# yandex/pire

Hardware: AMD Instinct MI355X
Metric: scanned GB/s (whole node) + ns/byte, 8-regex glued Scanner, 4KiB strings (higher is better)
Workload: dtype u8

## Files before the change

pire_amd/csrc/segmented.hip:

```cpp

#include <hip/hip_runtime.h>
#include <hipcub/hipcub.hpp>

#include <algorithm>
#include <cmath>
#include <chrono>
#include <cstdio>
#include <cstdlib>
#include <string>
#include <unordered_map>
#include <vector>

#include "device_common.h"

namespace pirehip {

namespace {

constexpr uint32_t kMaxModes = 6;
constexpr uint32_t kSlots = kMaxModes + 1;
constexpr uint64_t kResetMap = 1ull << 56;
constexpr uint32_t kNoSlot = 0xFF;
constexpr uint32_t kNoState = 0xFFFFFFFFu;

struct SegGeometry {
	uint64_t segBytes, warmBytes;
	uint64_t nStrings, nSeg;
	uint64_t segsPerString;
	const uint32_t* strFirst;
};

struct SegArrays {
	uint64_t* segBegin;
	uint64_t* segEnd;
	uint64_t* warmBegin;
	uint32_t* segStr;
	uint32_t* segJ;
	uint32_t* initSeg;
};

struct SlotArrays {
	uint32_t* guess[kSlots];
	uint32_t* end[kSlots];
	uint32_t count;
};

struct ChainArrays {
	uint64_t* prefix;
	uint32_t* trueStart;
	uint32_t* finalState;
	uint32_t* strDone;
	uint32_t* breakSeg;
	uint32_t* breakState;
	uint32_t* broken;
	uint64_t* blockAgg;
	uint64_t* blockPrefix;
	uint32_t* brokenHost;
};

__device__ __forceinline__ void StringOfSegment(const SegGeometry& g, uint64_t seg, uint64_t* str, uint64_t* j)
{
	if (!g.strFirst) {
		*str = seg / g.segsPerString;
		*j = seg - *str * g.segsPerString;
		return;
	}
	uint64_t lo = 0, hi = g.nStrings;
	while (hi - lo > 1) {
		const uint64_t mid = (lo + hi) / 2;
		if (g.strFirst[mid] <= seg)
			lo = mid;
		else
			hi = mid;
	}
	*str = lo;
	*j = seg - g.strFirst[lo];
}

__global__ void SegmentPrepKernel(ScanParams p, SegGeometry g, SegArrays a, uint32_t* patchGuess, uint32_t* patchEnd,
                                  uint32_t* strDone, uint32_t* breakSeg, uint32_t* broken)
{
	const uint64_t seg = uint64_t(blockIdx.x) * blockDim.x + threadIdx.x;
	if (seg >= g.nSeg)
		return;
	patchGuess[seg] = kNoState;
	patchEnd[seg] = kNoState;
	if (seg < g.nStrings) {
		strDone[seg] = 0;
		breakSeg[seg] = kNoState;
	}
	if (seg == 0)
		*broken = 0;
	uint64_t s, j;
	StringOfSegment(g, seg, &s, &j);
	uint64_t B, E;
	if (p.offsets) {
		B = p.offsets[s];
		E = p.offsets[s + 1];
	} else {
		B = s * p.stride;
		E = B + p.len;
	}
	const uint64_t b = B + j * g.segBytes;
	const uint64_t e = b + g.segBytes < E ? b + g.segBytes : E;
	const uint64_t w = j == 0 ? 0 : (b - B < g.warmBytes ? b - B : g.warmBytes);
	a.segBegin[seg] = b;
	a.segEnd[seg] = e;
	a.warmBegin[seg] = b - w;
	a.segStr[seg] = uint32_t(s);
	a.segJ[seg] = uint32_t(j);
	if (a.initSeg)
		a.initSeg[seg] = p.permOfOrig[p.initIdx[s]];
}

__global__ void SegmentFillKernel(uint32_t* dst, uint32_t value, uint64_t n)
{
	const uint64_t i = uint64_t(blockIdx.x) * blockDim.x + threadIdx.x;
	if (i < n)
		dst[i] = value;
}

__device__ __forceinline__ uint64_t MapOfSegment(const SegGeometry& g, const SegArrays& a, const SlotArrays& sl, uint64_t k)
{
	const bool last = k + 1 == g.nSeg || a.segJ[k + 1] == 0;
	uint64_t map = 0;
	if (!last) {
		uint32_t nextGuess[kSlots];
#pragma unroll
		for (uint32_t j = 0; j < kSlots; ++j)
			nextGuess[j] = (j < sl.count || j == kMaxModes) ? sl.guess[j][k + 1] : kNoState;
#pragma unroll
		for (uint32_t i = 0; i < kSlots; ++i) {
			uint32_t to = kNoSlot;
			if (i < sl.count || i == kMaxModes) {
				const uint32_t e = sl.end[i][k];
				const bool live = sl.guess[i][k] != kNoState;
#pragma unroll
				for (uint32_t j = kSlots; j-- > 0;)
					if (live && nextGuess[j] == e)
						to = j;
			}
			map |= uint64_t(to) << (8 * i);
		}
	}
	if (a.segJ[k] == 0) {
		const uint64_t to0 = map & 0xFF;
		map = to0 * 0x0001010101010101ull | kResetMap;
	}
	return map;
}

struct ComposeMaps {
	__host__ __device__ __forceinline__ uint64_t operator()(const uint64_t& first, const uint64_t& then) const
	{
		if (then & kResetMap)
			return then;
		uint64_t out = first & kResetMap;
#pragma unroll
		for (uint32_t i = 0; i < kSlots; ++i) {
			const uint32_t mid = uint32_t(first >> (8 * i)) & 0xFF;
			const uint32_t to = mid == kNoSlot ? kNoSlot : uint32_t(then >> (8 * mid)) & 0xFF;
			out |= uint64_t(to) << (8 * i);
		}
		return out;
	}
};

constexpr uint32_t kChainBlock = 1024;
constexpr uint64_t kIdentityMap = 0x0006050403020100ull;

__global__ __launch_bounds__(kChainBlock) void SegmentMapScanKernel(SegGeometry g, SegArrays a, SlotArrays sl, ChainArrays c)
{
	using Scan = hipcub::BlockScan<uint64_t, kChainBlock>;
	__shared__ typename Scan::TempStorage temp;
	const uint64_t k = uint64_t(blockIdx.x) * kChainBlock + threadIdx.x;
	uint64_t map = kIdentityMap;
	if (k < g.nSeg)
		map = MapOfSegment(g, a, sl, k);
	uint64_t incl;
	Scan(temp).InclusiveScan(map, incl, ComposeMaps());
	if (k < g.nSeg)
		c.prefix[k] = incl;
	if (threadIdx.x == kChainBlock - 1)
		c.blockAgg[blockIdx.x] = incl;
}

__global__ __launch_bounds__(kChainBlock) void SegmentBlockScanKernel(ChainArrays c, uint32_t nblocks)
{
	using Scan = hipcub::BlockScan<uint64_t, kChainBlock>;
	__shared__ typename Scan::TempStorage temp;
	__shared__ uint64_t next;
	uint64_t carry = kIdentityMap;
	for (uint32_t base = 0; base < nblocks; base += kChainBlock) {
		const uint32_t b = base + threadIdx.x;
		const uint64_t agg = b < nblocks ? c.blockAgg[b] : kIdentityMap;
		uint64_t in;
		Scan(temp).InclusiveScan(agg, in, ComposeMaps());
		const uint64_t out = ComposeMaps()(carry, in);
		if (b < nblocks)
			c.blockPrefix[b] = out;
		if (threadIdx.x == kChainBlock - 1)
			next = out;
		__syncthreads();
		carry = next;
		__syncthreads();
	}
}

__device__ __forceinline__ uint32_t ChainSlotAfter(const ChainArrays& c, uint64_t k)
{
	const uint64_t local = c.prefix[k];
// ... 147 lines not shown
						w = SlowStep(p, lds, L, w, byte);
						take(w);
					});
					hs = w < p.hot ? w : p.hot;
					cold = w;
				}
			}
			st = hs != p.hot ? hs : cold;
		}
		for (; q < qe; ++q) {
			st = SlowStep(p, lds, L, st, *q);
			take(st);
		}
		const bool last = k + 1 == g.nSeg || a.segJ[k + 1] == 0;
		if (last && (p.flags & PIRE_HIP_RUN_END)) {
			st = p.nextPerm[size_t(st) * p.letters + p.endCls];
			take(st);
		}
		const uint32_t str = a.segStr[k];
#pragma unroll
		for (int r = 0; r < 8; ++r)
			if (uint32_t(r) < p.regexps && c[r]) {
				if (str == firstStr)
					atomicAdd(&blockSum[r], c[r]);
				else
					atomicAdd(&results[size_t(str) * p.regexps + r], c[r]);
			}
	}
	__syncthreads();
	if (threadIdx.x < p.regexps && threadIdx.x < 8 && blockSum[threadIdx.x])
		atomicAdd(&results[size_t(firstStr) * p.regexps + threadIdx.x], blockSum[threadIdx.x]);
}

__global__ __launch_bounds__(256) void SegmentFinishSmallKernel(ScanParams p, const uint32_t* endIdx, const uint32_t* broken,
                                                               uint32_t* brokenHost)
{
	if (!ChainsIntact(broken, brokenHost))
		return;
	const uint64_t s = uint64_t(blockIdx.x) * blockDim.x + threadIdx.x;
	const bool active = s < p.n;
	const FinRec* recs = (p.flags & PIRE_HIP_RUN_END) ? p.finEnd : p.finSelf;
	u32x4 raw = {0, 0, 0, 0};
	if (active)
		raw = *reinterpret_cast<const u32x4*>(&recs[endIdx[s]]);
	const uint32_t orig = raw.x, endPerm = raw.y & 0x0FFFFFFFu, fl = raw.y >> 28;
	if (active) {
		if (p.outIdx)
			p.outIdx[s] = orig;
		if (p.outFinal)
			p.outFinal[s] = fl & kFinal;
	}
	if (!p.outCounts)
		return;
	const int lane = threadIdx.x & 63;
	const unsigned long long finals = __ballot(active && (fl & kFinal));
	const unsigned long long actives = __ballot(active);
	if (lane == 0 && actives) {
		atomicAdd(&p.outCounts[0], (unsigned long long)__popcll(finals));
		atomicAdd(&p.outCounts[1], (unsigned long long)__popcll(actives));
	}
	if (p.acceptMaskPerm) {
		const uint64_t m = active ? ((uint64_t(raw.w) << 32) | raw.z) : 0;
		if (__any(m != 0))
			for (uint32_t r = 0; r < p.regexps; ++r) {
				const unsigned long long b = __ballot((m >> r) & 1);
				if (lane == 0 && b)
					atomicAdd(&p.outCounts[2 + r], (unsigned long long)__popcll(b));
			}
	} else if (active) {
		for (uint64_t k = p.acceptOffPerm[endPerm]; k < p.acceptOffPerm[endPerm + 1]; ++k)
			atomicAdd(&p.outCounts[2 + p.acceptIds[k]], 1ull);
	}
}

uint64_t Knob(uint64_t v, uint64_t fallback)
{
	return v == 0 ? fallback : v == ~uint64_t(0) ? 0 : v;
}

struct HostWord {
	void* host = nullptr;
	uint32_t* dev = nullptr;
	size_t block = 0;
	int Acquire()
	{
		if (int rc = StagingAcquireHost(64, &host, &block))
			return rc;
		void* d = nullptr;
		const hipError_t e = hipHostGetDevicePointer(&d, host, 0);
		if (e != hipSuccess)
			return HipFail(e, "hipHostGetDevicePointer");
		dev = static_cast<uint32_t*>(d);
		return PIRE_HIP_OK;
	}
	~HostWord()
	{
		if (host)
			StagingReleaseHost(host, block);
	}
};

struct ScratchArena {
	StreamScratch block;
	uint8_t* base = nullptr;
	size_t size = 0, used = 0;
// ... 209 lines not shown
		prod.ranked = false;
		t->segProductA.resize(PN);
		t->segProductB.resize(PN);
		for (uint32_t i = 0; i < PN; ++i) {
			t->segProductA[i] = pairs[i].first;
			t->segProductB[i] = pairs[i].second;
		}
		t->segProduct.reset(new pire_hip_table);
		t->segProduct->host = std::move(prod);
	}
	if (t->segProduct && t->segProductA0 == a0 && t->segProductB0 == b0) {
		out->table = t->segProduct.get();
		out->compA = &t->segProductA;
		out->compB = &t->segProductB;
	}
	return PIRE_HIP_OK;
}

__global__ void SegmentSplitKernel(const uint32_t* guessP, const uint32_t* endP, const uint32_t* compA, const uint32_t* compB,
                                   uint32_t productStates, const uint32_t* productOrigOfPerm, const uint32_t* permOfOrig,
                                   uint32_t* guessA, uint32_t* endA, uint32_t* guessB, uint32_t* endB, uint64_t n)
{
	const uint64_t k = uint64_t(blockIdx.x) * blockDim.x + threadIdx.x;
	if (k >= n)
		return;
	const uint32_t g = guessP[k], e = endP[k];
	const uint32_t go = g < productStates ? productOrigOfPerm[g] : kNoState, eo = e < productStates ? productOrigOfPerm[e] : kNoState;
	guessA[k] = go != kNoState ? permOfOrig[compA[go]] : kNoState;
	guessB[k] = go != kNoState ? permOfOrig[compB[go]] : kNoState;
	endA[k] = eo != kNoState ? permOfOrig[compA[eo]] : kNoState;
	endB[k] = eo != kNoState ? permOfOrig[compB[eo]] : kNoState;
}

bool SegmentedEligible(uint64_t n, uint64_t totalBytes)
{
	const pire_hip_config cfg = GetConfig();
	if (cfg.no_segments || n == 0 || n >= (1ull << 20))
		return false;
	if (cfg.segment_bytes)
		return true;
	const double mean = double(totalBytes) / double(n);
	if (mean < 8192.0)
		return false;
	const double lanes = 256.0 * 1024.0;
	const double plain = std::ceil(double(n) / lanes) * mean / 25e6;
	const double segmented = double(totalBytes) / 2.0e12 + 80e-6;
	return plain > 1.5 * segmented;
}

int RunSegmented(pire_hip_table* t, const ScanParams& p, const uint64_t* hostOffsets, hipStream_t stream,
                 uint32_t* halfFinalResults, bool* halfFinalIncomplete)
{
	PIRE_TRY(CheckCounts(p));
	const pire_hip_config cfg = GetConfig();
	const bool wantStats = cfg.segment_stats != 0;
	auto t0 = std::chrono::steady_clock::now();
	std::string timeline;
	auto mark = [&](const char* what) {
		if (!wantStats)
			return;
		(void)hipStreamSynchronize(stream);
		const auto t1 = std::chrono::steady_clock::now();
		char buf[64];
		snprintf(buf, sizeof(buf), " %s %.0f us;", what, std::chrono::duration<double, std::micro>(t1 - t0).count());
		timeline += buf;
		t0 = t1;
	};
	const uint64_t n = p.n;
	const uint64_t total = hostOffsets ? hostOffsets[n] - hostOffsets[0] : n * p.len;
	int cus = 0;
	PIRE_TRY(DeviceCUs(&cus));
	const uint64_t wanted = uint64_t(cus) * 1024;
	uint64_t segBytes = std::min<uint64_t>(1u << 20, std::max<uint64_t>(1024, (total / wanted + 255) / 256 * 256));
	segBytes = Knob(cfg.segment_bytes, segBytes);
	const uint64_t warmBytes = Knob(cfg.segment_warmup, 256);
	const uint32_t maxModes = uint32_t(std::min<uint64_t>(kMaxModes, std::max<uint64_t>(1, Knob(cfg.segment_modes, 6))));
	uint64_t budget = Knob(cfg.segment_budget, 32);
	if (segBytes == 0) {
		SetError("PIRE_HIP_SEGMENT_BYTES must be positive");
		return PIRE_HIP_EINVAL;
	}

	SegGeometry g = {};
	g.segBytes = segBytes;
	g.warmBytes = warmBytes;
	g.nStrings = n;
	std::vector<uint32_t> strFirst(n + 1);
	{
		uint64_t acc = 0;
		for (uint64_t i = 0; i < n; ++i) {
			strFirst[i] = uint32_t(acc);
			const uint64_t len = hostOffsets ? hostOffsets[i + 1] - hostOffsets[i] : p.len;
			acc += std::max<uint64_t>(1, (len + segBytes - 1) / segBytes);
			if (acc >= (1ull << 31)) {
				SetError("too many segments");
				return PIRE_HIP_EINVAL;
			}
		}
		strFirst[n] = uint32_t(acc);
		g.nSeg = acc;
	}
	const uint64_t S = g.nSeg;
	ScratchArena scratch(stream);
	const uint64_t chainBlocks = (S + kChainBlock - 1) / kChainBlock;
	{
		const size_t perSeg = 3 * 8 + 3 * 4
		                      + (size_t(maxModes) + 1) * 8 + 4
		                      + 8
		                      + 4;
		const size_t perString = 5 * 4 + 2 * 8 + 3 * 4 + 4;
		PIRE_TRY(scratch.Reserve(S * perSeg + n * perString + chainBlocks * 16 + size_t(t->host.states) * 4 * kMaxModes + 64 * 256));
	}
	if (hostOffsets) {
		uint32_t* d = nullptr;
		PIRE_TRY(scratch.Alloc(&d, n + 1));
		PIRE_TRY(HipOk(hipMemcpyAsync(d, strFirst.data(), (n + 1) * 4, hipMemcpyHostToDevice, stream), "hipMemcpy(segment index)"));
		g.strFirst = d;
	} else {
		g.segsPerString = strFirst[1] - strFirst[0];
	}
	SegArrays a = {};
	PIRE_TRY(scratch.Alloc(&a.segBegin, S));
	PIRE_TRY(scratch.Alloc(&a.segEnd, S));
	PIRE_TRY(scratch.Alloc(&a.warmBegin, S));
	PIRE_TRY(scratch.Alloc(&a.segStr, S));
	PIRE_TRY(scratch.Alloc(&a.segJ, S));
	if (p.initIdx)
		PIRE_TRY(scratch.Alloc(&a.initSeg, S));
	const unsigned blocks = unsigned((S + 255) / 256);
	SlotArrays sl = {};
	PIRE_TRY(scratch.Alloc(&sl.guess[kMaxModes], S));
	PIRE_TRY(scratch.Alloc(&sl.end[kMaxModes], S));
	ChainArrays c = {};
	PIRE_TRY(scratch.Alloc(&c.prefix, S));
	PIRE_TRY(scratch.Alloc(&c.blockAgg, chainBlocks));
	PIRE_TRY(scratch.Alloc(&c.blockPrefix, chainBlocks));
	if (halfFinalResults)
		PIRE_TRY(scratch.Alloc(&c.trueStart, S));
	PIRE_TRY(scratch.Alloc(&c.finalState, n));
	PIRE_TRY(scratch.Alloc(&c.strDone, n));
	PIRE_TRY(scratch.Alloc(&c.breakSeg, n));
	PIRE_TRY(scratch.Alloc(&c.breakState, n));
	PIRE_TRY(scratch.Alloc(&c.broken, 1));
	auto segBeginOf = [&](uint64_t i, uint32_t k) {
		const uint64_t B = hostOffsets ? hostOffsets[i] : i * p.stride;
		return B + uint64_t(k - strFirst[i]) * segBytes;
	};
	auto stringEndOf = [&](uint64_t i) { return hostOffsets ? hostOffsets[i + 1] : i * p.stride + p.len; };

	ScanParams q = p;
	q.len = q.stride = 0;
	q.textEnd = hostOffsets ? hostOffsets[n] : (n - 1) * p.stride + p.len;
	q.outFinal = nullptr;
	q.outCounts = nullptr;

	uint64_t gridSegs = 0;
	if (!hostOffsets && !cfg.segment_no_grid) {
		if (n == 1)
			gridSegs = p.len / segBytes;
		else if (p.stride == p.len && p.len % segBytes == 0)
			gridSegs = S;
		ScanParams probe = q;
		probe.offsets = nullptr;
		probe.n = gridSegs;
		probe.len = probe.stride = segBytes;
		if (!TiledEligible(probe))
			gridSegs = 0;
	}

	uint32_t* dConst = nullptr;
	const uint64_t fusedSegs = (warmBytes % 256 == 0 && warmBytes <= segBytes && segBytes % 256 == 0 && !cfg.segment_no_pair)
	                               ? gridSegs & ~uint64_t(63) : 0;
	auto addMode = [&](bool first, uint32_t representative) -> int {
		const uint32_t m = sl.count;
		PIRE_TRY(scratch.Alloc(&sl.guess[m], S));
		PIRE_TRY(scratch.Alloc(&sl.end[m], S));
		if (fusedSegs) {
			ScanParams r = q;
			r.offsets = nullptr;
			r.ends = nullptr;
			r.n = fusedSegs;
			r.len = r.stride = segBytes;
			r.outIdx = sl.end[m];
			if (first) {
				r.initIdx = a.initSeg;
				r.flags = (p.flags & PIRE_HIP_RUN_BEGIN) | kPermIds;
			} else {
				r.initIdx = nullptr;
				r.startPerm = representative;
				r.flags = kPermIds;
			}
			PIRE_TRY(LaunchTiledSeg(r, warmBytes, a.segJ, sl.guess[m], stream));
			if (fusedSegs < S) {
				const uint64_t rest = S - fusedSegs;
				if (!first) {
					if (!dConst)
						PIRE_TRY(scratch.Alloc(&dConst, S));
					hipLaunchKernelGGL(SegmentFillKernel, dim3(unsigned((rest + 255) / 256)), dim3(256), 0, stream, dConst, representative, rest);
				}
				q.n = rest;
				q.offsets = a.warmBegin + fusedSegs;
				q.ends = a.segBegin + fusedSegs;
				q.initIdx = first ? (a.initSeg ? a.initSeg + fusedSegs : nullptr) : dConst;
				q.flags = (first ? (p.flags & PIRE_HIP_RUN_BEGIN) : 0u) | kPermIds;
				q.outIdx = sl.guess[m] + fusedSegs;
				PIRE_TRY(ScanBatch(q, t, stream));
				q.flags = kPermIds;
				q.offsets = a.segBegin + fusedSegs;
				q.ends = a.segEnd + fusedSegs;
				q.initIdx = sl.guess[m] + fusedSegs;
				q.outIdx = sl.end[m] + fusedSegs;
				PIRE_TRY(ScanBatch(q, t, stream));
			}
			sl.count = m + 1;
			return PIRE_HIP_OK;
		}
		q.n = S;
		q.offsets = a.warmBegin;
		q.ends = a.segBegin;
		if (first) {
			q.initIdx = a.initSeg;
			q.flags = (p.flags & PIRE_HIP_RUN_BEGIN) | kPermIds;
		} else {
			if (!dConst)
				PIRE_TRY(scratch.Alloc(&dConst, S));
			hipLaunchKernelGGL(SegmentFillKernel, dim3(blocks), dim3(256), 0, stream, dConst, representative, S);
			q.initIdx = dConst;
			q.flags = kPermIds;
		}
		q.outIdx = sl.guess[m];
		PIRE_TRY(ScanBatch(q, t, stream));
		q.flags = kPermIds;
		if (gridSegs) {
			ScanParams r = q;
			r.offsets = nullptr;
			r.ends = nullptr;
			r.n = gridSegs;
			r.len = r.stride = segBytes;
			r.initIdx = sl.guess[m];
			r.outIdx = sl.end[m];
			PIRE_TRY(LaunchTiled(r, stream));
		}
		if (gridSegs < S) {
			q.n = S - gridSegs;
			q.offsets = a.segBegin + gridSegs;
			q.ends = a.segEnd + gridSegs;
			q.initIdx = sl.guess[m] + gridSegs;
			q.outIdx = sl.end[m] + gridSegs;
			PIRE_TRY(ScanBatch(q, t, stream));
		}
		sl.count = m + 1;
		return PIRE_HIP_OK;
	};
	auto addModePair = [&](uint32_t representativeB) -> int {
		const uint32_t m = sl.count;
		for (uint32_t k = m; k < m + 2; ++k) {
			PIRE_TRY(scratch.Alloc(&sl.guess[k], S));
			PIRE_TRY(scratch.Alloc(&sl.end[k], S));
		}
		const uint64_t paired = gridSegs & ~uint64_t(63);
		const uint64_t separate = paired;
		if (separate < S) {
			if (!dConst)
				PIRE_TRY(scratch.Alloc(&dConst, S));
			hipLaunchKernelGGL(SegmentFillKernel, dim3(blocks), dim3(256), 0, stream, dConst, representativeB, S);
		}
		for (uint32_t k = 0; k < 2 && separate < S; ++k) {
			q.n = S - separate;
			q.offsets = a.warmBegin + separate;
			q.ends = a.segBegin + separate;
			q.initIdx = k == 0 ? (a.initSeg ? a.initSeg + separate : nullptr) : dConst;
			q.flags = (k == 0 ? (p.flags & PIRE_HIP_RUN_BEGIN) : 0u) | kPermIds;
			q.outIdx = sl.guess[m + k] + separate;
			PIRE_TRY(ScanBatch(q, t, stream));
		}
		q.flags = kPermIds;
		ScanParams ra = q;
		ra.offsets = nullptr;
		ra.ends = nullptr;
		ra.n = paired;
		ra.len = ra.stride = segBytes;
		ra.outIdx = sl.end[m];
		ScanParams rb = ra;
		ra.initIdx = a.initSeg;
		ra.flags = (p.flags & PIRE_HIP_RUN_BEGIN) | kPermIds;
		rb.initIdx = nullptr;
		rb.startPerm = representativeB;
		PIRE_TRY(LaunchPairTiled(ra, rb, sl.end[m + 1], stream, warmBytes, a.segJ, sl.guess[m], sl.guess[m + 1]));
		for (uint32_t k = 0; k < 2 && paired < S; ++k) {
			q.n = S - paired;
			q.offsets = a.segBegin + paired;
			q.ends = a.segEnd + paired;
			q.initIdx = sl.guess[m + k] + paired;
			q.outIdx = sl.end[m + k] + paired;
			PIRE_TRY(ScanBatch(q, t, stream));
		}
		sl.count = m + 2;
		return PIRE_HIP_OK;
	};
	StreamScratch productScratch(stream);
	void* pinnedComp = nullptr;
	size_t pinnedCompBytes = 0;
	struct PinnedCompGuard {
		void*& q;
		size_t& bytes;
		~PinnedCompGuard()
		{
			if (q)
				StagingReleaseHost(q, bytes);
		}
	} pinnedCompGuard{pinnedComp, pinnedCompBytes};
	bool productUsed = false;
	TableUse productUse;
	auto addModeProduct = [&](const ModeProduct& mp, uint32_t representativeB) -> int {
		const uint32_t m = sl.count;
		for (uint32_t k = m; k < m + 2; ++k) {
			PIRE_TRY(scratch.Alloc(&sl.guess[k], S));
			PIRE_TRY(scratch.Alloc(&sl.end[k], S));
		}
		ScanParams pp;
		PIRE_TRY(PrepareScanParams(mp.table, &pp, 0, &productUse));
		const HostTable& ph = mp.table->host;
		const uint32_t PN = ph.states;
		const size_t bytes = ((fusedSegs * 4 + 255) & ~size_t(255)) * 2 + ((size_t(PN) * 4 + 255) & ~size_t(255)) * 2;
		PIRE_TRY(productScratch.Alloc(bytes, "hipMallocAsync(product walk)"));
		uint8_t* base = productScratch.as<uint8_t>();
		uint32_t* guessP = reinterpret_cast<uint32_t*>(base);
		uint32_t* endP = reinterpret_cast<uint32_t*>(base + ((fusedSegs * 4 + 255) & ~size_t(255)));
		uint32_t* dCompA = reinterpret_cast<uint32_t*>(base + ((fusedSegs * 4 + 255) & ~size_t(255)) * 2);
		uint32_t* dCompB = dCompA + ((size_t(PN) + 63) & ~size_t(63));
		ScanParams r = pp;
		r.text = q.text;
		r.textEnd = q.textEnd;
		r.offsets = nullptr;
		r.ends = nullptr;
		r.n = fusedSegs;
		r.len = r.stride = segBytes;
		r.initIdx = nullptr;
		r.flags = kPermIds;
		r.outIdx = endP;
		r.outFinal = nullptr;
		r.outCounts = nullptr;
		PIRE_TRY(LaunchTiledSeg(r, warmBytes, a.segJ, guessP, stream));
		PIRE_TRY(StagingAcquireHost(size_t(PN) * 8, &pinnedComp, &pinnedCompBytes));
		uint32_t* hA = static_cast<uint32_t*>(pinnedComp);
		uint32_t* hB = hA + PN;
		memcpy(hA, mp.compA->data(), size_t(PN) * 4);
		memcpy(hB, mp.compB->data(), size_t(PN) * 4);
		PIRE_TRY(HipOk(hipMemcpyAsync(dCompA, hA, size_t(PN) * 4, hipMemcpyHostToDevice, stream), "hipMemcpy(product components)"));
		PIRE_TRY(HipOk(hipMemcpyAsync(dCompB, hB, size_t(PN) * 4, hipMemcpyHostToDevice, stream), "hipMemcpy(product components)"));
		hipLaunchKernelGGL(SegmentSplitKernel, dim3(unsigned((fusedSegs + 255) / 256)), dim3(256), 0, stream, guessP, endP, dCompA, dCompB,
		                   PN, pp.origOfPerm, p.permOfOrig, sl.guess[m], sl.end[m], sl.guess[m + 1], sl.end[m + 1], fusedSegs);
		if (fusedSegs < S) {
			const uint64_t rest = S - fusedSegs;
			if (!dConst)
				PIRE_TRY(scratch.Alloc(&dConst, S));
			hipLaunchKernelGGL(SegmentFillKernel, dim3(unsigned((rest + 255) / 256)), dim3(256), 0, stream, dConst, representativeB, rest);
			for (uint32_t k = 0; k < 2; ++k) {
				q.n = rest;
				q.offsets = a.warmBegin + fusedSegs;
				q.ends = a.segBegin + fusedSegs;
				q.initIdx = k == 0 ? nullptr : dConst;
				q.flags = (k == 0 ? (p.flags & PIRE_HIP_RUN_BEGIN) : 0u) | kPermIds;
				q.outIdx = sl.guess[m + k] + fusedSegs;
				PIRE_TRY(ScanBatch(q, t, stream));
				q.flags = kPermIds;
				q.offsets = a.segBegin + fusedSegs;
				q.ends = a.segEnd + fusedSegs;
				q.initIdx = sl.guess[m + k] + fusedSegs;
				q.outIdx = sl.end[m + k] + fusedSegs;
				PIRE_TRY(ScanBatch(q, t, stream));
			}
			q.flags = kPermIds;
		}
		productUsed = true;
		sl.count = m + 2;
		return PIRE_HIP_OK;
	};
	mark("setup");
	std::vector<uint32_t> known;
	{
		std::lock_guard<std::mutex> lock(t->segMutex);
		for (uint32_t r : t->segModes)
			if (r < t->host.states)
				known.push_back(r);
	}
	size_t nextKnown = 0;
	bool pairedFirst = false;
	if (!known.empty() && maxModes >= 2 && gridSegs >= 64 && !cfg.segment_no_pair && warmBytes % 256 == 0 && warmBytes <= segBytes) {
		ScanParams probe = q;
		probe.offsets = nullptr;
		probe.n = gridSegs & ~uint64_t(63);
		probe.len = probe.stride = segBytes;
		pairedFirst = TiledEligible(probe) && segBytes % 256 == 0;
	}
	hipLaunchKernelGGL(SegmentPrepKernel, dim3(blocks), dim3(256), 0, stream, p, g, a, sl.guess[kMaxModes], sl.end[kMaxModes],
	                   c.strDone, c.breakSeg, c.broken);
	const bool derive = !p.initIdx && !cfg.segment_no_derive && segBytes >= warmBytes && warmBytes < (1u << 20);
	const uint32_t minSteps = uint32_t(warmBytes);
	uint32_t a0 = t->host.initial;
	if (p.flags & PIRE_HIP_RUN_BEGIN)
		a0 = t->host.next[size_t(a0) * t->host.letters + t->host.cls[kBeginMark]];
	uint32_t* dModeFn = nullptr;
	void* pinnedFn = nullptr;
	size_t pinnedFnBytes = 0;
	struct PinnedGuard {
		void*& q;
		size_t& bytes;
		~PinnedGuard()
		{
			if (q)
				StagingReleaseHost(q, bytes);
		}
	} pinnedGuard{pinnedFn, pinnedFnBytes};
	uint32_t derivedModes = 0;
	auto addDerived = [&](const std::vector<uint32_t>& fOrig) -> int {
		const uint32_t m = sl.count;
		const uint32_t N = t->host.states;
		PIRE_TRY(scratch.Alloc(&sl.guess[m], S));
		PIRE_TRY(scratch.Alloc(&sl.end[m], S));
		if (!pinnedFn) {
			PIRE_TRY(StagingAcquireHost(size_t(N) * 4 * kMaxModes, &pinnedFn, &pinnedFnBytes));
			PIRE_TRY(scratch.Alloc(&dModeFn, size_t(N) * kMaxModes));
		}
		uint32_t* host = static_cast<uint32_t*>(pinnedFn) + size_t(derivedModes) * N;
		uint32_t* dev = dModeFn + size_t(derivedModes) * N;
		memcpy(host, fOrig.data(), size_t(N) * 4);
		PIRE_TRY(HipOk(hipMemcpyAsync(dev, host, size_t(N) * 4, hipMemcpyHostToDevice, stream), "hipMemcpy(mode function)"));
		hipLaunchKernelGGL(SegmentDeriveKernel, dim3(blocks), dim3(256), 0, stream, sl.guess[0], sl.end[0], dev, N, p.origOfPerm,
		                   p.permOfOrig, sl.guess[m], sl.end[m], S);
		++derivedModes;
		sl.count = m + 1;
		return PIRE_HIP_OK;
	};
	std::vector<std::vector<uint32_t>> derivable;
	std::vector<uint32_t> walked;
	for (uint32_t r : known) {
		std::vector<uint32_t> f;
		if (derive && derivable.size() + 1 < kMaxModes && ModeFunctionCached(t, a0, r, minSteps, &f))
			derivable.push_back(std::move(f));
		else
			walked.push_back(r);
	}
	ModeProduct product;
	if (pairedFirst && !walked.empty() && fusedSegs && !p.initIdx && !cfg.segment_no_product)
		PIRE_TRY(EnsureModeProduct(t, a0, walked[0], &product));
	if (product.table) {
		PIRE_TRY(addModeProduct(product, p.hostPermOfOrig[walked[0]]));
		nextKnown = 1;
		pairedFirst = false;
		mark("modes 0+1 (product)");
	} else if (pairedFirst && !walked.empty()) {
		PIRE_TRY(addModePair(p.hostPermOfOrig[walked[0]]));
		nextKnown = 1;
		mark("modes 0+1 (fused)");
	} else {
		pairedFirst = false;
		PIRE_TRY(addMode(true, 0));
		mark("mode 0");
	}
	for (const auto& f : derivable)
		if (sl.count < maxModes)
			PIRE_TRY(addDerived(f));
	for (; nextKnown < walked.size(); ++nextKnown)
		if (sl.count < maxModes)
			PIRE_TRY(addMode(false, p.hostPermOfOrig[walked[nextKnown]]));

	mark("known modes");
	HostWord brokenWord;
	PIRE_TRY(brokenWord.Acquire());
	c.brokenHost = brokenWord.dev;
	uint32_t *dExStr = nullptr, *dExInit = nullptr, *dExOut = nullptr;
	uint64_t *dExB = nullptr, *dExE = nullptr;
	std::vector<uint32_t> breakSeg(n), breakState(n), exStr, exInit;
	std::vector<uint64_t> exB, exE;
	std::unordered_map<uint32_t, uint32_t> surprises;
	uint64_t nWalked = 0, nPlain = 0, rounds = 0;
	auto launchFinish = [&](const uint32_t* broken) -> int {
		if (n <= 4096) {
			hipLaunchKernelGGL(SegmentFinishSmallKernel, dim3(unsigned((n + 255) / 256)), dim3(256), 0, stream, p, c.finalState, broken,
			                   c.brokenHost);
		} else {
			ScanParams f = p;
			f.compact = 0;
			const LdsLayout L = MakeLayout(f.hot, f.outCounts ? f.regexps : 0, kRotPitch, 0);
			PIRE_TRY(HipOk(SetDynamicLds(reinterpret_cast<const void*>(SegmentFinishKernel), uint32_t(L.total)), "hipFuncSetAttribute(LDS)"));
			const unsigned threads = 1024;
			const uint64_t tasks = (n + 63) / 64;
			const unsigned cblocks = unsigned(std::max<uint64_t>(1, std::min<uint64_t>((tasks * 64 + threads - 1) / threads, uint64_t(cus))));
			hipLaunchKernelGGL(SegmentFinishKernel, dim3(cblocks), dim3(threads), L.total, stream, f, c.finalState, broken, c.brokenHost);
		}
		return PIRE_HIP_OK;
	};
	for (;;) {
		++rounds;
		*static_cast<volatile uint32_t*>(brokenWord.host) = kNoState;
		hipLaunchKernelGGL(SegmentMapScanKernel, dim3(unsigned(chainBlocks)), dim3(kChainBlock), 0, stream, g, a, sl, c);
		if (chainBlocks > 1)
			hipLaunchKernelGGL(SegmentBlockScanKernel, dim3(1), dim3(kChainBlock), 0, stream, c, uint32_t(chainBlocks));
		hipLaunchKernelGGL(SegmentResolveKernel, dim3(blocks), dim3(256), 0, stream, g, a, sl, c);
		if (halfFinalResults)
			hipLaunchKernelGGL(SegmentReportKernel, dim3(1), dim3(64), 0, stream, c.broken, c.brokenHost);
		else
			PIRE_TRY(launchFinish(c.broken));
		PIRE_TRY(HipOk(hipGetLastError(), "segmented scan: chain kernels"));
		PIRE_TRY(HipOk(hipStreamSynchronize(stream), "hipStreamSynchronize"));
		const uint32_t broken = *static_cast<volatile uint32_t*>(brokenWord.host);
		if (broken == kNoState) {
			SetError("segmented scan: the chain kernels did not report");
			return PIRE_HIP_EUNSUPPORTED;
		}
		if (!broken)
			break;
		PIRE_TRY(HipOk(hipMemsetAsync(c.broken, 0, 4, stream), "hipMemset"));
		PIRE_TRY(HipOk(hipMemcpyAsync(breakSeg.data(), c.breakSeg, n * 4, hipMemcpyDeviceToHost, stream), "hipMemcpy(D2H)"));
		PIRE_TRY(HipOk(hipMemcpyAsync(breakState.data(), c.breakState, n * 4, hipMemcpyDeviceToHost, stream), "hipMemcpy(D2H)"));
		PIRE_TRY(HipOk(hipStreamSynchronize(stream), "hipStreamSynchronize"));
		exStr.clear();
		for (uint64_t i = 0; i < n; ++i)
			if (breakSeg[i] != kNoState && breakSeg[i] > strFirst[i] && breakSeg[i] < strFirst[i + 1])
				exStr.push_back(uint32_t(i));
		if (exStr.size() != broken) {
			SetError("segmented scan: inconsistent chain state");
			return PIRE_HIP_EUNSUPPORTED;
		}
		uint32_t best = 0, bestCount = 0;
		{
			std::vector<uint32_t> seen;
			for (uint32_t i : exStr)
				seen.push_back(breakState[i]);
			std::sort(seen.begin(), seen.end());
			seen.erase(std::unique(seen.begin(), seen.end()), seen.end());
			for (uint32_t v : seen) {
				const uint32_t cnt = ++surprises[v];
				if (cnt > bestCount) {
					best = v;
					bestCount = cnt;
				}
			}
		}
		if (sl.count < maxModes && (bestCount >= 2 || budget == 0)) {
			std::vector<uint32_t> f;
			if (derive && derivedModes + 1 < kMaxModes && ModeFunctionCached(t, a0, p.hostOrigOfPerm[best], minSteps, &f))
				PIRE_TRY(addDerived(f));
			else
				PIRE_TRY(addMode(false, best));
// ... 8 lines not shown
			continue;
		}
		const bool plain = budget == 0;
		if (!plain)
			--budget;
		const size_t m = exStr.size();
		exB.resize(m);
		exE.resize(m);
		exInit.resize(m);
		for (size_t j = 0; j < m; ++j) {
			const uint64_t i = exStr[j];
			exB[j] = segBeginOf(i, breakSeg[i]);
			exE[j] = plain ? stringEndOf(i) : std::min(stringEndOf(i), exB[j] + segBytes);
			exInit[j] = breakState[i];
		}
		if (!dExB) {
			PIRE_TRY(scratch.Alloc(&dExB, n));
			PIRE_TRY(scratch.Alloc(&dExE, n));
			PIRE_TRY(scratch.Alloc(&dExStr, n));
			PIRE_TRY(scratch.Alloc(&dExInit, n));
			PIRE_TRY(scratch.Alloc(&dExOut, n));
		}
		PIRE_TRY(HipOk(hipMemcpyAsync(dExB, exB.data(), m * 8, hipMemcpyHostToDevice, stream), "hipMemcpy(H2D)"));
		PIRE_TRY(HipOk(hipMemcpyAsync(dExE, exE.data(), m * 8, hipMemcpyHostToDevice, stream), "hipMemcpy(H2D)"));
		PIRE_TRY(HipOk(hipMemcpyAsync(dExStr, exStr.data(), m * 4, hipMemcpyHostToDevice, stream), "hipMemcpy(H2D)"));
		PIRE_TRY(HipOk(hipMemcpyAsync(dExInit, exInit.data(), m * 4, hipMemcpyHostToDevice, stream), "hipMemcpy(H2D)"));
		q.n = m;
		q.offsets = dExB;
		q.ends = dExE;
		q.initIdx = dExInit;
		q.flags = kPermIds;
		q.outIdx = dExOut;
		PIRE_TRY(ScanBatch(q, t, stream));
		hipLaunchKernelGGL(SegmentPatchKernel, dim3(unsigned((m + 255) / 256)), dim3(256), 0, stream, dExStr, dExOut, uint32_t(m),
		                   plain ? 1u : 0u, sl, c);
		PIRE_TRY(HipOk(hipMemsetAsync(c.breakSeg, 0xFF, n * 4, stream), "hipMemset"));
		PIRE_TRY(HipOk(hipStreamSynchronize(stream), "hipStreamSynchronize"));
		(plain ? nPlain : nWalked) += m;
	}

	mark("chain");
	if (halfFinalIncomplete)
		*halfFinalIncomplete = nPlain != 0;
	if (halfFinalResults && !nPlain) {
		PIRE_TRY(HipOk(hipMemsetAsync(halfFinalResults, 0, n * size_t(p.regexps) * 4, stream), "hipMemset"));
		ScanParams hp = p;
		hp.compact = 0;
		const LdsLayout L = MakeLayout(hp.hot, 0, 256u, 0);
		const uint32_t ldsBytes = L.total + 64;
		PIRE_TRY(HipOk(SetDynamicLds(reinterpret_cast<const void*>(SegmentHalfFinalKernel), uint32_t(ldsBytes)), "hipFuncSetAttribute(LDS)"));
		const uint32_t initialPerm = p.hostPermOfOrig[t->host.initial];
		hipLaunchKernelGGL(SegmentHalfFinalKernel, dim3(unsigned((S + 1023) / 1024)), dim3(1024), ldsBytes, stream, hp, g, a,
		                   c.trueStart, c.strDone, initialPerm, halfFinalResults);
		mark("half-final counts");
	}
	if (halfFinalResults)
		PIRE_TRY(launchFinish(nullptr));
	PIRE_TRY(HipOk(hipGetLastError(), "segmented scan launch"));
	NoteKernel(nPlain ? "segmented+plain" : "segmented",
	           pairedFirst ? "pirehip::ScanPairTiledKernel"
	           : productUsed ? "pirehip::ScanTiledSegKernel+product"
	           : fusedSegs   ? (derivedModes ? "pirehip::ScanTiledSegKernel+derived" : "pirehip::ScanTiledSegKernel")
	                         : "");
	if (wantStats) {
		mark("finish");
		fprintf(stderr, "pire_hip segmented: %llu strings, %llu segments of %llu B (+%llu B warm-up), %u modes, %llu chain "
		                "rounds; segments scanned again from the chain's state %llu, strings left to the plain walk %llu;%s\n",
		        (unsigned long long)n, (unsigned long long)S, (unsigned long long)segBytes, (unsigned long long)warmBytes,
		        sl.count, (unsigned long long)rounds, (unsigned long long)nWalked, (unsigned long long)nPlain, timeline.c_str());
	}
	return PIRE_HIP_OK;
}

}
```

Before: 6472.

## Fuse chain resolve, finish and product split into fewer segmented-scan kernel launches

Adds a single SegmentChainKernel that recomputes block prefixes per block, resolves each segment's slot and, for small batches, runs the per-string finish inline, replacing the block-scan, resolve and finish launches. It also folds the product-state split into the map-scan kernel via a by-value component table, which avoids a pinned host copy, two H2D copies and the split kernel. Segment size is now picked by a cost model that trades walk length against warm-up rescans. The aim is to cut launch and latency overhead for short scans, at the cost of a larger kernel argument, redundant per-block prefix scans, and added complexity in the broken-chain reporting.

```diff
diff --git a/pire_amd/csrc/segmented.hip b/pire_amd/csrc/segmented.hip
--- a/pire_amd/csrc/segmented.hip
+++ b/pire_amd/csrc/segmented.hip
@@ -56,6 +56,7 @@
 	uint64_t* blockAgg;
 	uint64_t* blockPrefix;
 	uint32_t* brokenHost;
+	uint32_t* finished;
 };
 
 __device__ __forceinline__ void StringOfSegment(const SegGeometry& g, uint64_t seg, uint64_t* str, uint64_t* j)
@@ -78,7 +79,7 @@
 }
 
 __global__ void SegmentPrepKernel(ScanParams p, SegGeometry g, SegArrays a, uint32_t* patchGuess, uint32_t* patchEnd,
-                                  uint32_t* strDone, uint32_t* breakSeg, uint32_t* broken)
+                                  uint32_t* strDone, uint32_t* breakSeg, uint32_t* broken, uint32_t* finished)
 {
 	const uint64_t seg = uint64_t(blockIdx.x) * blockDim.x + threadIdx.x;
 	if (seg >= g.nSeg)
@@ -88,6 +89,7 @@
 	if (seg < g.nStrings) {
 		strDone[seg] = 0;
 		breakSeg[seg] = kNoState;
+		finished[seg] = 0;
 	}
 	if (seg == 0)
 		*broken = 0;
@@ -120,21 +122,53 @@
 		dst[i] = value;
 }
 
-__device__ __forceinline__ uint64_t MapOfSegment(const SegGeometry& g, const SegArrays& a, const SlotArrays& sl, uint64_t k)
+constexpr uint32_t kFoldStates = 448;
+struct ProductFold {
+	uint64_t segs;
+	const uint32_t* guessP;
+	const uint32_t* endP;
+	const uint32_t* origOfPerm;
+	const uint32_t* permOfOrig;
+	uint32_t states;
+	uint16_t compA[kFoldStates], compB[kFoldStates];
+};
+
+__device__ __forceinline__ void SplitProductState(const ProductFold& pf, uint32_t s, uint32_t* sa, uint32_t* sb)
+{
+	const uint32_t o = s < pf.states ? pf.origOfPerm[s] : kNoState;
+	*sa = o != kNoState ? pf.permOfOrig[pf.compA[o]] : kNoState;
+	*sb = o != kNoState ? pf.permOfOrig[pf.compB[o]] : kNoState;
+}
+
+__device__ __forceinline__ uint64_t MapOfSegment(const SegGeometry& g, const SegArrays& a, const SlotArrays& sl, uint64_t k,
+                                                 const ProductFold& pf)
 {
 	const bool last = k + 1 == g.nSeg || a.segJ[k + 1] == 0;
+	uint32_t ownGuess[2] = {0, 0}, ownEnd[2] = {0, 0};
+	const bool folded = k < pf.segs;
+	if (folded) {
+		SplitProductState(pf, pf.guessP[k], &ownGuess[0], &ownGuess[1]);
+		SplitProductState(pf, pf.endP[k], &ownEnd[0], &ownEnd[1]);
+#pragma unroll
+		for (uint32_t i = 0; i < 2; ++i) {
+			sl.guess[i][k] = ownGuess[i];
+			sl.end[i][k] = ownEnd[i];
+		}
+	}
 	uint64_t map = 0;
 	if (!last) {
 		uint32_t nextGuess[kSlots];
 #pragma unroll
 		for (uint32_t j = 0; j < kSlots; ++j)
-			nextGuess[j] = (j < sl.count || j == kMaxModes) ? sl.guess[j][k + 1] : kNoState;
+			nextGuess[j] = (j < sl.count || j == kMaxModes) && !(j < 2 && k + 1 < pf.segs) ? sl.guess[j][k + 1] : kNoState;
+		if (k + 1 < pf.segs)
+			SplitProductState(pf, pf.guessP[k + 1], &nextGuess[0], &nextGuess[1]);
 #pragma unroll
 		for (uint32_t i = 0; i < kSlots; ++i) {
 			uint32_t to = kNoSlot;
 			if (i < sl.count || i == kMaxModes) {
-				const uint32_t e = sl.end[i][k];
-				const bool live = sl.guess[i][k] != kNoState;
+				const uint32_t e = i < 2 && folded ? ownEnd[i & 1] : sl.end[i][k];
+				const bool live = (i < 2 && folded ? ownGuess[i & 1] : sl.guess[i][k]) != kNoState;
 #pragma unroll
 				for (uint32_t j = kSlots; j-- > 0;)
 					if (live && nextGuess[j] == e)
@@ -169,14 +203,15 @@
 constexpr uint32_t kChainBlock = 1024;
 constexpr uint64_t kIdentityMap = 0x0006050403020100ull;
 
-__global__ __launch_bounds__(kChainBlock) void SegmentMapScanKernel(SegGeometry g, SegArrays a, SlotArrays sl, ChainArrays c)
+__global__ __launch_bounds__(kChainBlock) void SegmentMapScanKernel(SegGeometry g, SegArrays a, SlotArrays sl, ChainArrays c,
+                                                                    ProductFold pf)
 {
 	using Scan = hipcub::BlockScan<uint64_t, kChainBlock>;
 	__shared__ typename Scan::TempStorage temp;
 	const uint64_t k = uint64_t(blockIdx.x) * kChainBlock + threadIdx.x;
 	uint64_t map = kIdentityMap;
 	if (k < g.nSeg)
-		map = MapOfSegment(g, a, sl, k);
+		map = MapOfSegment(g, a, sl, k, pf);
 	uint64_t incl;
 	Scan(temp).InclusiveScan(map, incl, ComposeMaps());
 	if (k < g.nSeg)
@@ -390,17 +425,12 @@
 		atomicAdd(&results[size_t(firstStr) * p.regexps + threadIdx.x], blockSum[threadIdx.x]);
 }
 
-__global__ __launch_bounds__(256) void SegmentFinishSmallKernel(ScanParams p, const uint32_t* endIdx, const uint32_t* broken,
-                                                               uint32_t* brokenHost)
-{
-	if (!ChainsIntact(broken, brokenHost))
-		return;
-	const uint64_t s = uint64_t(blockIdx.x) * blockDim.x + threadIdx.x;
-	const bool active = s < p.n;
+__device__ __forceinline__ void FinishString(const ScanParams& p, uint64_t s, bool active, uint32_t endState)
+{
 	const FinRec* recs = (p.flags & PIRE_HIP_RUN_END) ? p.finEnd : p.finSelf;
 	u32x4 raw = {0, 0, 0, 0};
 	if (active)
-		raw = *reinterpret_cast<const u32x4*>(&recs[endIdx[s]]);
+		raw = *reinterpret_cast<const u32x4*>(&recs[endState]);
 	const uint32_t orig = raw.x, endPerm = raw.y & 0x0FFFFFFFu, fl = raw.y >> 28;
 	if (active) {
 		if (p.outIdx)
@@ -429,6 +459,88 @@
 		for (uint64_t k = p.acceptOffPerm[endPerm]; k < p.acceptOffPerm[endPerm + 1]; ++k)
 			atomicAdd(&p.outCounts[2 + p.acceptIds[k]], 1ull);
 	}
+}
+
+__global__ __launch_bounds__(256) void SegmentFinishSmallKernel(ScanParams p, const uint32_t* endIdx, const uint32_t* broken,
+                                                               uint32_t* brokenHost)
+{
+	if (!ChainsIntact(broken, brokenHost))
+		return;
+	const uint64_t s = uint64_t(blockIdx.x) * blockDim.x + threadIdx.x;
+	const bool active = s < p.n;
+	FinishString(p, s, active, active ? endIdx[s] : 0u);
+}
+
+constexpr uint32_t kChainMaxBlocks = kChainBlock;
+
+__global__ __launch_bounds__(kChainBlock) void SegmentChainKernel(ScanParams p, SegGeometry g, SegArrays a, SlotArrays sl,
+                                                                  ChainArrays c, uint32_t finish)
+{
+	using Scan = hipcub::BlockScan<uint64_t, kChainBlock>;
+	__shared__ typename Scan::TempStorage temp;
+	__shared__ uint32_t enter[2];
+	const uint32_t b = blockIdx.x;
+	if (threadIdx.x < 2)
+		enter[threadIdx.x] = 0;
+	__syncthreads();
+	if (b) {
+		const uint64_t agg = threadIdx.x < b ? c.blockAgg[threadIdx.x] : kIdentityMap;
+		uint64_t in;
+		Scan(temp).InclusiveScan(agg, in, ComposeMaps());
+		if (threadIdx.x + 1 == b)
+			enter[1] = uint32_t(in) & 0xFF;
+		if (threadIdx.x + 2 == b)
+			enter[0] = uint32_t(in) & 0xFF;
+		__syncthreads();
+	}
+	auto slotAfter = [&](uint64_t kk) -> uint32_t {
+		const uint64_t local = c.prefix[kk];
+		const uint64_t bb = kk / kChainBlock;
+		if (bb == 0 || (local & kResetMap))
+			return uint32_t(local) & 0xFF;
+		const uint32_t mid = bb == b ? enter[1] : enter[0];
+		return mid == kNoSlot ? kNoSlot : uint32_t(local >> (8 * mid)) & 0xFF;
+	};
+	const uint64_t k = uint64_t(b) * kChainBlock + threadIdx.x;
+	bool ends = false;
+	uint32_t str = 0, st = 0;
+	if (k < g.nSeg) {
+		str = a.segStr[k];
+		const bool last = k + 1 == g.nSeg || a.segJ[k + 1] == 0;
+		if (c.strDone[str]) {
+			ends = last;
+			st = c.finalState[str];
+		} else {
+			const uint32_t j = a.segJ[k];
+			const uint32_t slot = j == 0 ? 0u : slotAfter(k - 1);
+			if (slot == kNoSlot) {
+				const uint32_t before = j == 1 ? 0u : slotAfter(k - 2);
+				if (before != kNoSlot) {
+					c.breakSeg[str] = uint32_t(k);
+					c.breakState[str] = sl.end[before][k - 1];
+					atomicAdd(c.broken, 1u);
+					__hip_atomic_store(c.brokenHost, 1u, __ATOMIC_RELAXED, __HIP_MEMORY_SCOPE_SYSTEM);
+				}
+			} else {
+				if (c.trueStart)
+					c.trueStart[k] = sl.guess[slot][k];
+				if (last) {
+					st = sl.end[slot][k];
+					c.finalState[str] = st;
+					ends = true;
+				}
+			}
+		}
+	}
+	if (!finish)
+		return;
+	if (ends) {
+		if (c.finished[str])
+			ends = false;
+		else
+			c.finished[str] = 1;
+	}
+	FinishString(p, str, ends, st);
 }
 
 uint64_t Knob(uint64_t v, uint64_t fallback)
@@ -704,6 +816,27 @@
 	endB[k] = eo != kNoState ? permOfOrig[compB[eo]] : kNoState;
 }
 
+constexpr double kStepSeconds = 42e-9;
+constexpr double kPassRate = 6.1e12;
+
+static uint64_t ChooseSegmentBytes(uint64_t total, uint64_t lanes, uint64_t warmBytes)
+{
+	const uint64_t fill = std::min<uint64_t>(1u << 20, std::max<uint64_t>(256, (total / lanes + 255) / 256 * 256));
+	const uint64_t least = std::max<uint64_t>(256, (warmBytes + 255) / 256 * 256);
+	uint64_t best = std::max(fill, least);
+	double bestCost = 0;
+	for (uint64_t seg = least; seg <= fill; seg += 256) {
+		const double segs = std::ceil(double(total) / double(seg));
+		const double walk = std::ceil(segs / double(lanes)) * double(seg + warmBytes) * kStepSeconds;
+		const double again = double(warmBytes) / double(seg) * double(total) / kPassRate;
+		if (seg == least || walk + again < bestCost) {
+			best = seg;
+			bestCost = walk + again;
+		}
+	}
+	return best;
+}
+
 bool SegmentedEligible(uint64_t n, uint64_t totalBytes)
 {
 	const pire_hip_config cfg = GetConfig();
@@ -716,7 +849,7 @@
 		return false;
 	const double lanes = 256.0 * 1024.0;
 	const double plain = std::ceil(double(n) / lanes) * mean / 25e6;
-	const double segmented = double(totalBytes) / 2.0e12 + 80e-6;
+	const double segmented = double(totalBytes) / 2.0e12 + 75e-6;
 	return plain > 1.5 * segmented;
 }
 
@@ -739,13 +872,13 @@
 		t0 = t1;
 	};
 	const uint64_t n = p.n;
+	uint32_t launches = 0;
 	const uint64_t total = hostOffsets ? hostOffsets[n] - hostOffsets[0] : n * p.len;
 	int cus = 0;
 	PIRE_TRY(DeviceCUs(&cus));
 	const uint64_t wanted = uint64_t(cus) * 1024;
-	uint64_t segBytes = std::min<uint64_t>(1u << 20, std::max<uint64_t>(1024, (total / wanted + 255) / 256 * 256));
-	segBytes = Knob(cfg.segment_bytes, segBytes);
 	const uint64_t warmBytes = Knob(cfg.segment_warmup, 256);
+	uint64_t segBytes = Knob(cfg.segment_bytes, ChooseSegmentBytes(total, wanted, warmBytes));
 	const uint32_t maxModes = uint32_t(std::min<uint64_t>(kMaxModes, std::max<uint64_t>(1, Knob(cfg.segment_modes, 6))));
 	uint64_t budget = Knob(cfg.segment_budget, 32);
 	if (segBytes == 0) {
@@ -780,7 +913,7 @@
 		                      + (size_t(maxModes) + 1) * 8 + 4
 		                      + 8
 		                      + 4;
-		const size_t perString = 5 * 4 + 2 * 8 + 3 * 4 + 4;
+		const size_t perString = 6 * 4 + 2 * 8 + 3 * 4 + 4;
 		PIRE_TRY(scratch.Reserve(S * perSeg + n * perString + chainBlocks * 16 + size_t(t->host.states) * 4 * kMaxModes + 64 * 256));
 	}
 	if (hostOffsets) {
@@ -814,6 +947,7 @@
 	PIRE_TRY(scratch.Alloc(&c.breakSeg, n));
 	PIRE_TRY(scratch.Alloc(&c.breakState, n));
 	PIRE_TRY(scratch.Alloc(&c.broken, 1));
+	PIRE_TRY(scratch.Alloc(&c.finished, n));
 	auto segBeginOf = [&](uint64_t i, uint32_t k) {
 		const uint64_t B = hostOffsets ? hostOffsets[i] : i * p.stride;
 		return B + uint64_t(k - strFirst[i]) * segBytes;
@@ -863,12 +997,14 @@
 				r.flags = kPermIds;
 			}
 			PIRE_TRY(LaunchTiledSeg(r, warmBytes, a.segJ, sl.guess[m], stream));
+			++launches;
 			if (fusedSegs < S) {
 				const uint64_t rest = S - fusedSegs;
 				if (!first) {
 					if (!dConst)
 						PIRE_TRY(scratch.Alloc(&dConst, S));
 					hipLaunchKernelGGL(SegmentFillKernel, dim3(unsigned((rest + 255) / 256)), dim3(256), 0, stream, dConst, representative, rest);
+					++launches;
 				}
 				q.n = rest;
 				q.offsets = a.warmBegin + fusedSegs;
@@ -877,12 +1013,14 @@
 				q.flags = (first ? (p.flags & PIRE_HIP_RUN_BEGIN) : 0u) | kPermIds;
 				q.outIdx = sl.guess[m] + fusedSegs;
 				PIRE_TRY(ScanBatch(q, t, stream));
+				++launches;
 				q.flags = kPermIds;
 				q.offsets = a.segBegin + fusedSegs;
 				q.ends = a.segEnd + fusedSegs;
 				q.initIdx = sl.guess[m] + fusedSegs;
 				q.outIdx = sl.end[m] + fusedSegs;
 				PIRE_TRY(ScanBatch(q, t, stream));
+				++launches;
 			}
 			sl.count = m + 1;
 			return PIRE_HIP_OK;
@@ -897,11 +1035,13 @@
 			if (!dConst)
 				PIRE_TRY(scratch.Alloc(&dConst, S));
 			hipLaunchKernelGGL(SegmentFillKernel, dim3(blocks), dim3(256), 0, stream, dConst, representative, S);
+			++launches;
 			q.initIdx = dConst;
 			q.flags = kPermIds;
 		}
 		q.outIdx = sl.guess[m];
 		PIRE_TRY(ScanBatch(q, t, stream));
+		++launches;
 		q.flags = kPermIds;
 		if (gridSegs) {
 			ScanParams r = q;
@@ -912,6 +1052,7 @@
 			r.initIdx = sl.guess[m];
 			r.outIdx = sl.end[m];
 			PIRE_TRY(LaunchTiled(r, stream));
+			++launches;
 		}
 		if (gridSegs < S) {
 			q.n = S - gridSegs;
@@ -920,6 +1061,7 @@
 			q.initIdx = sl.guess[m] + gridSegs;
 			q.outIdx = sl.end[m] + gridSegs;
 			PIRE_TRY(ScanBatch(q, t, stream));
+			++launches;
 		}
 		sl.count = m + 1;
 		return PIRE_HIP_OK;
@@ -936,6 +1078,7 @@
 			if (!dConst)
 				PIRE_TRY(scratch.Alloc(&dConst, S));
 			hipLaunchKernelGGL(SegmentFillKernel, dim3(blocks), dim3(256), 0, stream, dConst, representativeB, S);
+			++launches;
 		}
 		for (uint32_t k = 0; k < 2 && separate < S; ++k) {
 			q.n = S - separate;
@@ -945,6 +1088,7 @@
 			q.flags = (k == 0 ? (p.flags & PIRE_HIP_RUN_BEGIN) : 0u) | kPermIds;
 			q.outIdx = sl.guess[m + k] + separate;
 			PIRE_TRY(ScanBatch(q, t, stream));
+			++launches;
 		}
 		q.flags = kPermIds;
 		ScanParams ra = q;
@@ -959,6 +1103,7 @@
 		rb.initIdx = nullptr;
 		rb.startPerm = representativeB;
 		PIRE_TRY(LaunchPairTiled(ra, rb, sl.end[m + 1], stream, warmBytes, a.segJ, sl.guess[m], sl.guess[m + 1]));
+		++launches;
 		for (uint32_t k = 0; k < 2 && paired < S; ++k) {
 			q.n = S - paired;
 			q.offsets = a.segBegin + paired;
@@ -966,6 +1111,7 @@
 			q.initIdx = sl.guess[m + k] + paired;
 			q.outIdx = sl.end[m + k] + paired;
 			PIRE_TRY(ScanBatch(q, t, stream));
+			++launches;
 		}
 		sl.count = m + 2;
 		return PIRE_HIP_OK;
@@ -984,7 +1130,8 @@
 	} pinnedCompGuard{pinnedComp, pinnedCompBytes};
 	bool productUsed = false;
 	TableUse productUse;
-	auto addModeProduct = [&](const ModeProduct& mp, uint32_t representativeB) -> int {
+	ProductFold fold = {};
+	auto addModeProduct = [&](const ModeProduct& mp, uint32_t representativeB, bool foldSplit) -> int {
 		const uint32_t m = sl.count;
 		for (uint32_t k = m; k < m + 2; ++k) {
 			PIRE_TRY(scratch.Alloc(&sl.guess[k], S));
@@ -1014,6 +1161,19 @@
 		r.outFinal = nullptr;
 		r.outCounts = nullptr;
 		PIRE_TRY(LaunchTiledSeg(r, warmBytes, a.segJ, guessP, stream));
+		++launches;
+		if (foldSplit && PN <= kFoldStates && t->host.states <= 0xFFFF) {
+			fold.segs = fusedSegs;
+			fold.guessP = guessP;
+			fold.endP = endP;
+			fold.origOfPerm = pp.origOfPerm;
+			fold.permOfOrig = p.permOfOrig;
+			fold.states = PN;
+			for (uint32_t i = 0; i < PN; ++i) {
+				fold.compA[i] = uint16_t((*mp.compA)[i]);
+				fold.compB[i] = uint16_t((*mp.compB)[i]);
+			}
+		} else {
 		PIRE_TRY(StagingAcquireHost(size_t(PN) * 8, &pinnedComp, &pinnedCompBytes));
 		uint32_t* hA = static_cast<uint32_t*>(pinnedComp);
 		uint32_t* hB = hA + PN;
@@ -1023,11 +1183,14 @@
 		PIRE_TRY(HipOk(hipMemcpyAsync(dCompB, hB, size_t(PN) * 4, hipMemcpyHostToDevice, stream), "hipMemcpy(product components)"));
 		hipLaunchKernelGGL(SegmentSplitKernel, dim3(unsigned((fusedSegs + 255) / 256)), dim3(256), 0, stream, guessP, endP, dCompA, dCompB,
 		                   PN, pp.origOfPerm, p.permOfOrig, sl.guess[m], sl.end[m], sl.guess[m + 1], sl.end[m + 1], fusedSegs);
+		launches += 3;
+		}
 		if (fusedSegs < S) {
 			const uint64_t rest = S - fusedSegs;
 			if (!dConst)
 				PIRE_TRY(scratch.Alloc(&dConst, S));
 			hipLaunchKernelGGL(SegmentFillKernel, dim3(unsigned((rest + 255) / 256)), dim3(256), 0, stream, dConst, representativeB, rest);
+			++launches;
 			for (uint32_t k = 0; k < 2; ++k) {
 				q.n = rest;
 				q.offsets = a.warmBegin + fusedSegs;
@@ -1036,12 +1199,14 @@
 				q.flags = (k == 0 ? (p.flags & PIRE_HIP_RUN_BEGIN) : 0u) | kPermIds;
 				q.outIdx = sl.guess[m + k] + fusedSegs;
 				PIRE_TRY(ScanBatch(q, t, stream));
+				++launches;
 				q.flags = kPermIds;
 				q.offsets = a.segBegin + fusedSegs;
 				q.ends = a.segEnd + fusedSegs;
 				q.initIdx = sl.guess[m + k] + fusedSegs;
 				q.outIdx = sl.end[m + k] + fusedSegs;
 				PIRE_TRY(ScanBatch(q, t, stream));
+				++launches;
 			}
 			q.flags = kPermIds;
 		}
@@ -1067,7 +1232,8 @@
 		pairedFirst = TiledEligible(probe) && segBytes % 256 == 0;
 	}
 	hipLaunchKernelGGL(SegmentPrepKernel, dim3(blocks), dim3(256), 0, stream, p, g, a, sl.guess[kMaxModes], sl.end[kMaxModes],
-	                   c.strDone, c.breakSeg, c.broken);
+	                   c.strDone, c.breakSeg, c.broken, c.finished);
+	++launches;
 	const bool derive = !p.initIdx && !cfg.segment_no_derive && segBytes >= warmBytes && warmBytes < (1u << 20);
 	const uint32_t minSteps = uint32_t(warmBytes);
 	uint32_t a0 = t->host.initial;
@@ -1101,6 +1267,7 @@
 		PIRE_TRY(HipOk(hipMemcpyAsync(dev, host, size_t(N) * 4, hipMemcpyHostToDevice, stream), "hipMemcpy(mode function)"));
 		hipLaunchKernelGGL(SegmentDeriveKernel, dim3(blocks), dim3(256), 0, stream, sl.guess[0], sl.end[0], dev, N, p.origOfPerm,
 		                   p.permOfOrig, sl.guess[m], sl.end[m], S);
+		++launches;
 		++derivedModes;
 		sl.count = m + 1;
 		return PIRE_HIP_OK;
@@ -1118,7 +1285,7 @@
 	if (pairedFirst && !walked.empty() && fusedSegs && !p.initIdx && !cfg.segment_no_product)
 		PIRE_TRY(EnsureModeProduct(t, a0, walked[0], &product));
 	if (product.table) {
-		PIRE_TRY(addModeProduct(product, p.hostPermOfOrig[walked[0]]));
+		PIRE_TRY(addModeProduct(product, p.hostPermOfOrig[walked[0]], derivable.empty()));
 		nextKnown = 1;
 		pairedFirst = false;
 		mark("modes 0+1 (product)");
@@ -1148,6 +1315,7 @@
 	std::vector<uint64_t> exB, exE;
 	std::unordered_map<uint32_t, uint32_t> surprises;
 	uint64_t nWalked = 0, nPlain = 0, rounds = 0;
+	uint32_t firstRoundLaunches = 0;
 	auto launchFinish = [&](const uint32_t* broken) -> int {
 		if (n <= 4096) {
 			hipLaunchKernelGGL(SegmentFinishSmallKernel, dim3(unsigned((n + 255) / 256)), dim3(256), 0, stream, p, c.finalState, broken,
@@ -1166,24 +1334,36 @@
 	};
 	for (;;) {
 		++rounds;
-		*static_cast<volatile uint32_t*>(brokenWord.host) = kNoState;
-		hipLaunchKernelGGL(SegmentMapScanKernel, dim3(unsigned(chainBlocks)), dim3(kChainBlock), 0, stream, g, a, sl, c);
-		if (chainBlocks > 1)
+		*static_cast<volatile uint32_t*>(brokenWord.host) = 0;
+		hipLaunchKernelGGL(SegmentMapScanKernel, dim3(unsigned(chainBlocks)), dim3(kChainBlock), 0, stream, g, a, sl, c, fold);
+		fold.segs = 0;
+		++launches;
+		if (chainBlocks <= kChainMaxBlocks) {
+			const bool finishHere = !halfFinalResults && n <= 4096;
+			hipLaunchKernelGGL(SegmentChainKernel, dim3(unsigned(chainBlocks)), dim3(kChainBlock), 0, stream, p, g, a, sl, c,
+			                   finishHere ? 1u : 0u);
+			++launches;
+			if (!halfFinalResults && !finishHere) {
+				PIRE_TRY(launchFinish(c.broken));
+				++launches;
+			}
+		} else {
 			hipLaunchKernelGGL(SegmentBlockScanKernel, dim3(1), dim3(kChainBlock), 0, stream, c, uint32_t(chainBlocks));
-		hipLaunchKernelGGL(SegmentResolveKernel, dim3(blocks), dim3(256), 0, stream, g, a, sl, c);
-		if (halfFinalResults)
-			hipLaunchKernelGGL(SegmentReportKernel, dim3(1), dim3(64), 0, stream, c.broken, c.brokenHost);
-		else
-			PIRE_TRY(launchFinish(c.broken));
+			hipLaunchKernelGGL(SegmentResolveKernel, dim3(blocks), dim3(256), 0, stream, g, a, sl, c);
+			if (halfFinalResults)
+				hipLaunchKernelGGL(SegmentReportKernel, dim3(1), dim3(64), 0, stream, c.broken, c.brokenHost);
+			else
+				PIRE_TRY(launchFinish(c.broken));
+			launches += 3;
+		}
 		PIRE_TRY(HipOk(hipGetLastError(), "segmented scan: chain kernels"));
+		if (rounds == 1)
+			firstRoundLaunches = launches;
 		PIRE_TRY(HipOk(hipStreamSynchronize(stream), "hipStreamSynchronize"));
-		const uint32_t broken = *static_cast<volatile uint32_t*>(brokenWord.host);
-		if (broken == kNoState) {
-			SetError("segmented scan: the chain kernels did not report");
-			return PIRE_HIP_EUNSUPPORTED;
-		}
-		if (!broken)
+		if (!*static_cast<volatile uint32_t*>(brokenWord.host))
 			break;
+		uint32_t broken = 0;
+		PIRE_TRY(HipOk(hipMemcpyAsync(&broken, c.broken, 4, hipMemcpyDeviceToHost, stream), "hipMemcpy(D2H)"));
 		PIRE_TRY(HipOk(hipMemsetAsync(c.broken, 0, 4, stream), "hipMemset"));
 		PIRE_TRY(HipOk(hipMemcpyAsync(breakSeg.data(), c.breakSeg, n * 4, hipMemcpyDeviceToHost, stream), "hipMemcpy(D2H)"));
 		PIRE_TRY(HipOk(hipMemcpyAsync(breakState.data(), c.breakState, n * 4, hipMemcpyDeviceToHost, stream), "hipMemcpy(D2H)"));
@@ -1258,6 +1438,7 @@
 		q.flags = kPermIds;
 		q.outIdx = dExOut;
 		PIRE_TRY(ScanBatch(q, t, stream));
+		++launches;
 		hipLaunchKernelGGL(SegmentPatchKernel, dim3(unsigned((m + 255) / 256)), dim3(256), 0, stream, dExStr, dExOut, uint32_t(m),
 		                   plain ? 1u : 0u, sl, c);
 		PIRE_TRY(HipOk(hipMemsetAsync(c.breakSeg, 0xFF, n * 4, stream), "hipMemset"));
@@ -1291,9 +1472,9 @@
 	if (wantStats) {
 		mark("finish");
 		fprintf(stderr, "pire_hip segmented: %llu strings, %llu segments of %llu B (+%llu B warm-up), %u modes, %llu chain "
-		                "rounds; segments scanned again from the chain's state %llu, strings left to the plain walk %llu;%s\n",
+		                "rounds, %u launches in front of the first synchronise; segments scanned again from the chain's state %llu, strings left to the plain walk %llu;%s\n",
 		        (unsigned long long)n, (unsigned long long)S, (unsigned long long)segBytes, (unsigned long long)warmBytes,
-		        sl.count, (unsigned long long)rounds, (unsigned long long)nWalked, (unsigned long long)nPlain, timeline.c_str());
+		        sl.count, (unsigned long long)rounds, firstRoundLaunches, (unsigned long long)nWalked, (unsigned long long)nPlain, timeline.c_str());
 	}
 	return PIRE_HIP_OK;
 }
```

New measurement: 6462. Within noise of the previous version (-0.2%).
